# Maofei/loam_velodyne-1

Hardware: AMD Instinct MI355X
Metric: scans/sec (odometry+mapping L-M solve) VLP-16 sweep, 1/2/4/8 MI355X (higher is better)
Workload: dtype fp32 (fp64 JtJ accumulation); 1 GPU; config4: independent VLP-16 problems (SR prev+cur, odometry L-M, mapping L-M); problems_per_gpu=1024, global_batch=1024, split=strong, parallelism=shard1

## Files before the change

### loam_velodyne-1_amd/csrc/dev_common.hpp

```cpp
#ifndef LOAM_DEV_COMMON_HPP
#define LOAM_DEV_COMMON_HPP

#include <hip/hip_runtime.h>
#include <stdint.h>

#define LOAM_HD __host__ __device__ __forceinline__
#define LOAM_D __device__ __forceinline__

#ifdef LOAM_BOUNDS_CHECK
#define LOAM_CHECK(cond, a, b)                                                                      \
  do {                                                                                              \
    if (!(cond)) printf("LOAM_CHECK %s:%d %s (%lld, %lld)\n", __FILE__, __LINE__, #cond, (long long)(a), \
                        (long long)(b));                                                            \
  } while (0)
#else
#define LOAM_CHECK(cond, a, b) ((void)0)
#endif

struct PhaseAcc {
  unsigned long long s0, s1, s2;
  unsigned long long sum[2][12];
};
#ifdef LOAM_PHASES
#define LOAM_PH(...) __VA_ARGS__
// ... 362 lines not shown
    for (int stride = size >> 1; stride > 0; stride >>= 1) {
      for (int t = threadIdx.x; t < (n64 >> 1); t += NT) {
        int lo = 2 * t - (t & (stride - 1));
        int hi = lo + stride;
        bool up = ((lo & size) == 0);
        uint64_t a = k[lo], b = k[hi];
        if ((a > b) == up) { k[lo] = b; k[hi] = a; }
      }
      const int next = stride > 1 ? stride >> 1 : (size << 1 <= n64 ? size : 0);
      if (stride > 64 || next > 64 || next == 0) {
        __syncthreads();
      } else {
        __threadfence_block();
        __builtin_amdgcn_wave_barrier();
      }
    }
  }
}

LOAM_D uint64_t shfl_xor_u64(uint64_t v, int m) {
  const int lo = __shfl_xor((int)(uint32_t)v, m, 64), hi = __shfl_xor((int)(uint32_t)(v >> 32), m, 64);
  return ((uint64_t)(uint32_t)hi << 32) | (uint32_t)lo;
}
template <int E, int S>
LOAM_D void reg_cmpx_intra(uint64_t (&v)[E], int base, int size) {
#pragma unroll
  for (int e = 0; e < E; ++e) {
    if constexpr (S < E) {
      if ((e & S) == 0) {
        const bool up = ((base + e) & size) == 0;
        const uint64_t a = v[e], b = v[e + S];
        const bool sw = (a > b) == up;
        v[e] = sw ? b : a;
        v[e + S] = sw ? a : b;
      }
    }
  }
}
template <int NT, int E, bool WAVE = false>
LOAM_D void reg_bitonic_sort_n(uint64_t* k, int n) {
  static_assert(!WAVE || NT == 64, "a wave sort has 64 lanes");
  const int lane = __lane_id(), tid = WAVE ? lane : (int)threadIdx.x, base = tid * E;
  constexpr int N = NT * E;
  uint64_t v[E];
#pragma unroll
  for (int e = 0; e < E; ++e) {
    const int g = e * NT + tid;
    v[e] = g < n ? k[g] : ~0ull;
  }
  if (!WAVE) __syncthreads();
  for (int size = 2; size <= N; size <<= 1) {
    for (int stride = size >> 1; stride > 0; stride >>= 1) {
      if (stride < E) {
        if (stride == 1) reg_cmpx_intra<E, 1>(v, base, size);
        else if (stride == 2) reg_cmpx_intra<E, 2>(v, base, size);
        else if (stride == 4) reg_cmpx_intra<E, 4>(v, base, size);
        else reg_cmpx_intra<E, 8>(v, base, size);
      } else if (stride < 64 * E) {
        const int m = stride / E;
        const bool lower = (lane & m) == 0;
#pragma unroll
        for (int e = 0; e < E; ++e) {
          const bool up = ((base + e) & size) == 0;
          const uint64_t o = shfl_xor_u64(v[e], m);
          const bool keep_min = lower == up;
          v[e] = keep_min ? (o < v[e] ? o : v[e]) : (o > v[e] ? o : v[e]);
        }
      } else {
        const int m = stride / E;
        const bool lower = (tid & m) == 0;
#pragma unroll
        for (int e = 0; e < E; ++e) k[e * NT + tid] = v[e];
        __syncthreads();
#pragma unroll
        for (int e = 0; e < E; ++e) {
          const bool up = ((base + e) & size) == 0;
          const uint64_t o = k[e * NT + (tid ^ m)];
          const bool keep_min = lower == up;
          v[e] = keep_min ? (o < v[e] ? o : v[e]) : (o > v[e] ? o : v[e]);
        }
        __syncthreads();
      }
    }
  }
  if (WAVE) __builtin_amdgcn_wave_barrier();
#pragma unroll
  for (int e = 0; e < E; ++e)
    if (base + e < n) k[base + e] = v[e];
  if (WAVE) {
    __threadfence_block();
    __builtin_amdgcn_wave_barrier();
  } else {
    __syncthreads();
  }
}
LOAM_D void wave_sort_u64(uint64_t* k, int n) {
  if (n <= 64) reg_bitonic_sort_n<64, 1, true>(k, n);
  else if (n <= 128) reg_bitonic_sort_n<64, 2, true>(k, n);
  else if (n <= 256) reg_bitonic_sort_n<64, 4, true>(k, n);
  else reg_bitonic_sort_n<64, 8, true>(k, n);
}
template <int NT, int EMAX>
LOAM_D void reg_bitonic_sort(uint64_t* k, int n) {
  if (n <= NT || EMAX == 1) reg_bitonic_sort_n<NT, 1>(k, n);
  else if (n <= 2 * NT || EMAX == 2) reg_bitonic_sort_n<NT, (EMAX < 2 ? EMAX : 2)>(k, n);
  else if (n <= 4 * NT || EMAX == 4) reg_bitonic_sort_n<NT, (EMAX < 4 ? EMAX : 4)>(k, n);
  else if (n <= 8 * NT || EMAX == 8) reg_bitonic_sort_n<NT, (EMAX < 8 ? EMAX : 8)>(k, n);
  else reg_bitonic_sort_n<NT, (EMAX < 16 ? EMAX : 16)>(k, n);
}

template <int NT, int E>
LOAM_D int block_radix_sort_kv(uint32_t* ka, uint16_t* va, uint32_t* kb, uint16_t* vb, int n, int nbits,
                               uint32_t* sc) {
  constexpr int NW = NT / 64;
  const int tid = threadIdx.x, lane = __lane_id(), w = tid >> 6;
  int cur = 0;
  for (int shift = 0; shift < nbits; shift += 4) {
    const uint32_t* ks = cur ? kb : ka;
    const uint16_t* vs = cur ? vb : va;
    uint32_t* kd = cur ? ka : kb;
    uint16_t* vd = cur ? va : vb;
    uint32_t k[E];
    uint32_t meta[E];
    uint64_t clo = 0, chi = 0;
#pragma unroll
    for (int e = 0; e < E; ++e) {
      const int g = tid * E + e;
      k[e] = 0;
      meta[e] = 0;
      if (g < n) {
        k[e] = ks[g];
// ... 813 lines not shown
```

### loam_velodyne-1_amd/csrc/engine.hpp

```cpp
#ifndef LOAM_ENGINE_HPP
#define LOAM_ENGINE_HPP

#include <hip/hip_runtime.h>
#include <stdint.h>

#include <cstring>
#include <string>

#include "../../include/loam/loam.h"
#include "imu.hpp"
#include "prof.hpp"

namespace loam {

enum : int {
  ERR_CAP_RING = 1,
  ERR_CAP_ROWS = 2,
  ERR_EMPTY = 4,
  ERR_CAP_MAP = 8,
  ERR_CAP_STACK = 16,
  ERR_VG_BITS = 32,
};

constexpr int kSrThreads = 512;
// ... 50 lines not shown
      if (std::strcmp(key, k.n) == 0) {
        if (read) {
          *read = *k.f;
          return true;
        }
        if (v < k.lo || v > k.hi) return false;
        *k.f = (int)v;
        return true;
      }
    return false;
  }
};

struct SrBuffers {
  int S = 0, cap = 0, R = 0;
  float4* raw = nullptr;
  int* raw_n = nullptr;
  float* tmp_ori = nullptr;
  uint8_t* tmp_sid = nullptr;
  int* tilecnt = nullptr;
  int* tileF = nullptr;
  int* ring_sync = nullptr;
  float* sweep_ori = nullptr;
  float4* full = nullptr;
  int* n_full = nullptr;
  float* curv = nullptr;
  uint8_t* picked = nullptr;
  int* sortind = nullptr;
  int8_t* label = nullptr;
  int* ring_se = nullptr;
  int* st_sharp = nullptr;
  int* st_lsharp = nullptr;
  int* st_flat = nullptr;
  float4* st_lflat = nullptr;
  int* st_cnt = nullptr;
  uint16_t* st_cand = nullptr;
  int* st_ncand = nullptr;
  float4* sharp = nullptr;
  float4* lsharp = nullptr;
  float4* flat = nullptr;
  float4* lflat = nullptr;
  int* cnt = nullptr;
  int* err = nullptr;
  int* sel_big = nullptr;
  int* sel_list = nullptr;
  int* st_loff = nullptr;
// ... 133 lines not shown
```

### loam_velodyne-1_amd/csrc/sr.hip

```cpp
#include <cmath>
#include <type_traits>
#include <vector>

#include "dev_common.hpp"
#include "dev_hooks.h"
#include "engine.hpp"

using namespace loamdev;

namespace loam {

#ifdef LOAM_SR_PHASES
__device__ unsigned long long g_sr_ph[8];
#define SR_PH(k)                                                                  \
  do {                                                                            \
    if (threadIdx.x == 0) {                                                       \
      const unsigned long long now = __builtin_amdgcn_s_memrealtime();            \
      ph_t[k] = now - ph_last;                                                    \
      ph_last = now;                                                              \
    }                                                                             \
  } while (0)
#else
#define SR_PH(k) ((void)0)
#endif

namespace {


LOAM_HD int ring_id(const SrParams& p, float angle) {
  if (p.ring_model == LOAM_RING_LINEAR) {
    const float step = (p.ring_hi - p.ring_lo) / (float)(p.R - 1);
    const float angleID = (angle - p.ring_lo) / step;
    return (int)(angleID + 0.5f);
  }
  int rounded = (int)(D(angle) + (D(angle) < 0.0 ? -0.5 : +0.5));
  return rounded > 0 ? rounded : rounded + (p.R - 1);
}

LOAM_D int ring_of_exact(const SrParams& p, float px, float py, float pz) {
  const float af = atanf(py / sqrtf(px * px + pz * pz)) * 57.2957795f;
  const int lo = ring_id(p, af - 1e-3f), hi = ring_id(p, af + 1e-3f);
  if (lo == hi) return lo;
  return ring_id(p, (float)(atan(D(py) / sqrt(D(px * px + pz * pz))) * 180 / M_PI));
}

#ifndef LOAM_SR_RING_TAB
// ... 510 lines not shown
          T.valid = 1;
        }
      }
    }
    return;
  }
#pragma unroll
  for (int e = 0; e < kRingE; ++e) {
    const int i = t * kRingTile + e * kSrThreads + tid;
    if (sid[e] != 255) {
      const int pos = sh_base[sid[e]] + sh_pre[sid[e]] + sh_wcnt[sid[e]][e * kW + w] + rank[e];
      const float o = (i <= F) ? ori_first(ori[e], startOri) : ori_second(ori[e], endOri);
      const float relTime = (o - startOri) / (endOri - startOri);
      b.full[(size_t)s * b.cap + pos] = make_float4(q[e].y, q[e].z, q[e].x, (float)(sid[e] + 0.1 * D(relTime)));
    }
  }
}

#ifndef LOAM_SR_RING_FUSED
#define LOAM_SR_RING_FUSED 1
#endif
constexpr bool kSrRingFused = LOAM_SR_RING_FUSED;
constexpr int kSrRingFusedMin = 64;
__global__ __launch_bounds__(kSrThreads) void k_sr_ring_fused(SrBuffers b, SrParams p, int rtiles) {
  constexpr int kW = kSrThreads / 64, kSlots = kRingE * kW;
  static_assert(kSlots <= 64 && (kSlots & (kSlots - 1)) == 0, "slot scan width");
  const int tid = threadIdx.x, lane = lane_id(), w = tid >> 6;
  __shared__ int sh_ticket, sh_last, sh_F;
  __shared__ float sh_start, sh_end_raw;
  __shared__ int sh_cnt[64], sh_tot[64], sh_pre[64], sh_base[64];
  __shared__ int sh_wcnt[64][kSlots];
#ifdef LOAM_SR_PHASES
  unsigned long long ph_t[8] = {0}, ph_last = __builtin_amdgcn_s_memrealtime();
#endif
  if (tid == 0) sh_ticket = atomicAdd(&b.ring_sync[0], 1);
  __syncthreads();
  SR_PH(1);
  const int s = sh_ticket / rtiles, t = sh_ticket % rtiles;
  const int n = b.raw_n[s], R = p.R, nt = (n + kRingTile - 1) / kRingTile;
  const int nb = key_bits(R);
  if (t == 0) {
    if (tid < 2 * R) b.ring_se[s * 2 * R + tid] = 0;
    if (tid == 0) b.err[s] = 0;
  }
  if (n <= 0) {
    if (t == 0 && tid == 0) {
      b.n_full[s] = 0;
      b.err[s] |= ERR_EMPTY;
    }
    return;
  }
  if (t >= nt) return;
  const float4* raw = b.raw + (size_t)s * b.cap;
  float4 q[kRingE];
#pragma unroll
  for (int e = 0; e < kRingE; ++e) {
    const int i = t * kRingTile + e * kSrThreads + tid;
    q[e] = i < n ? raw[i] : make_float4(0, 0, 0, 0);
  }
  if (w < 2) {
    int f = -1;
    float4 v = make_float4(0, 0, 0, 0);
    for (int k = 0; k < n; k += 64) {
      const int i = w == 0 ? k + lane : n - 1 - k - lane;
      const bool in = w == 0 ? i < n : i >= 0;
      v = in ? raw[i] : make_float4(0, 0, 0, 0);
      const uint64_t m = __ballot(in && finite3(v));
      if (m) {
        const int src = __ffsll((unsigned long long)m) - 1;
        f = w == 0 ? k + src : n - 1 - k - src;
        v.x = __shfl(v.x, src, 64);
        v.y = __shfl(v.y, src, 64);
        break;
      }
    }
    if (lane == 0) {
      if (w == 0) {
        sh_start = f >= 0 ? -atan2f_fdlibm(v.y, v.x) : 0.0f;
      } else {
        sh_last = f;
        if (f >= 0) sh_end_raw = -atan2f_fdlibm(v.y, v.x);
      }
    }
  }
  __shared__ float4 sh_rtab[kRingTabMax];
  ring_tab_load(p, sh_rtab);
  if (tid < R) sh_cnt[tid] = 0;
  if (tid == 0) sh_F = 0x7fffffff;
  for (int k = tid; k < 64 * kSlots; k += kSrThreads) (&sh_wcnt[0][0])[k] = 0;
  __syncthreads();
  SR_PH(2);
  const float startOri = sh_start;
  float endOri = 0.0f;
  if (sh_last >= 0) {
    endOri = (float)(D(sh_end_raw) + 2 * M_PI);
    if (D(endOri - startOri) > 3 * M_PI) endOri = (float)(D(endOri) - 2 * M_PI);
    else if (D(endOri - startOri) < M_PI) endOri = (float)(D(endOri) + 2 * M_PI);
  }
  if (tid == 0 && t == 0) {
    if (sh_last < 0) b.err[s] |= ERR_EMPTY;
    b.sweep_ori[2 * s] = startOri;
    b.sweep_ori[2 * s + 1] = endOri;
  }
  int sid[kRingE], rank[kRingE];
  float ori[kRingE];
  int Floc = 0x7fffffff;
#pragma unroll
  for (int e = 0; e < kRingE; ++e) {
    const int i = t * kRingTile + e * kSrThreads + tid;
    sid[e] = 255;
    ori[e] = 0.0f;
    if (i < n && finite3(q[e])) {
      const float px = q[e].y, py = q[e].z, pz = q[e].x;
      const int scanID = ring_of(p, sh_rtab, px, py, pz);
      if (scanID >= 0 && scanID <= R - 1) {
        sid[e] = scanID;
        ori[e] = -atan2f_fdlibm(px, pz);
        if (D(ori_first(ori[e], startOri) - startOri) > M_PI) Floc = min(Floc, i);
        atomicAdd(&sh_cnt[scanID], 1);
      }
    }
  }
  Floc = wave_min_i(Floc);
// ... 175 lines not shown
  uint64_t keys[CAP];
  int sidx[SIDX ? CAP : 1];
  uint16_t cand[CAP];
  uint8_t pk[CAP + 16];
  int8_t lab[CAP + 16];
  int se[128];
  int picks[kSharpPerRing + kLessSharpPerRing + kFlatPerRing];
  int scratch[16];
  float red[6][kSelThreads / 64];
  int order[64];
  int nsharp, nlsharp, nflat, ncand, wf, big, loff;
};

#ifndef LOAM_RINGVG_PAD
#define LOAM_RINGVG_PAD 0
#endif
#ifndef LOAM_VG_GATHER
#define LOAM_VG_GATHER 4
#endif
constexpr int kVgGather = LOAM_VG_GATHER;
#ifndef LOAM_RINGVG_HOLD
#define LOAM_RINGVG_HOLD 1
#endif
template <int CAP, bool BIG, typename CandT>
LOAM_D int ring_vg(const float4* pts, int lo, const CandT* cand, int nc, uint64_t* keys, float4* outp, int outcap,
                   float (*red)[kSelThreads / 64], int* scratch, int* err) {
  const int tid = threadIdx.x, lane = lane_id(), w = tid >> 6;
  float mn[3] = {3.4e38f, 3.4e38f, 3.4e38f}, mx[3] = {-3.4e38f, -3.4e38f, -3.4e38f};
  constexpr bool HOLD = !BIG && CAP <= 2048 && LOAM_RINGVG_HOLD;
  constexpr int RH = HOLD ? CAP / kSelThreads : 1;
  float4 held[RH];
  if constexpr (HOLD) {
#pragma unroll
    for (int e = 0; e < RH; ++e) {
      const int t = e * kSelThreads + tid;
      held[e] = t < nc ? pts[lo + cand[t]] : make_float4(0, 0, 0, 0);
    }
#pragma unroll
    for (int e = 0; e < RH; ++e)
      if (e * kSelThreads + tid < nc) {
        const float4 a = held[e];
        mn[0] = fminf(mn[0], a.x); mn[1] = fminf(mn[1], a.y); mn[2] = fminf(mn[2], a.z);
        mx[0] = fmaxf(mx[0], a.x); mx[1] = fmaxf(mx[1], a.y); mx[2] = fmaxf(mx[2], a.z);
      }
  } else {
    for (int t = tid; t < nc; t += kSelThreads) {
      const float4 a = pts[lo + cand[t]];
      mn[0] = fminf(mn[0], a.x); mn[1] = fminf(mn[1], a.y); mn[2] = fminf(mn[2], a.z);
      mx[0] = fmaxf(mx[0], a.x); mx[1] = fmaxf(mx[1], a.y); mx[2] = fmaxf(mx[2], a.z);
    }
  }
  for (int d = 0; d < 3; ++d) {
    mn[d] = wave_min_f_x(mn[d]);
    mx[d] = wave_max_f_x(mx[d]);
    if (lane == 0) { red[d][w] = mn[d]; red[3 + d][w] = mx[d]; }
  }
  __syncthreads();
  for (int d = 0; d < 3; ++d)
    for (int v = 0; v < kSelThreads / 64; ++v) {
      mn[d] = fminf(mn[d], red[d][v]);
      mx[d] = fmaxf(mx[d], red[3 + d][v]);
    }
  __syncthreads();
  int nout = 0;
  if (nc > 0) {
    const float inv = 1.0f / 0.2f;
    if (vg_leaf_too_small(mn, mx, inv)) {
      for (int t = tid; t < nc; t += kSelThreads)
        if (t < outcap) outp[t] = pts[lo + cand[t]];
      nout = nc;
    } else {
      int minb[3], maxb[3];
      for (int d = 0; d < 3; ++d) {
        minb[d] = (int)floorf(mn[d] * inv);
        maxb[d] = (int)floorf(mx[d] * inv);
      }
      const int divx = maxb[0] - minb[0] + 1, divy = maxb[1] - minb[1] + 1;
      const int mul1 = divx, mul2 = divx * divy;
      if constexpr (!BIG) {
        constexpr int NW = kSelThreads / 64;
        int nruns = 0;
        if constexpr (HOLD) {
          static_assert(RH * NW <= 64, "slot prefix over one wave");
          __shared__ uint32_t rs_edge[RH * NW];
          __shared__ int rs_cnt[RH * NW];
          uint32_t idx[RH];
          int ex[RH];
#pragma unroll
          for (int e = 0; e < RH; ++e) {
            const int t = e * kSelThreads + tid;
            idx[e] = 0xffffffffu;
            if (t < nc) {
              const float4 a = held[e];
              const int i0 = (int)(floorf(a.x * inv) - (float)minb[0]);
              const int i1 = (int)(floorf(a.y * inv) - (float)minb[1]);
              const int i2 = (int)(floorf(a.z * inv) - (float)minb[2]);
              idx[e] = (uint32_t)(i0 + i1 * mul1 + i2 * mul2);
            }
            if (lane == 63) rs_edge[e * NW + w] = idx[e];
          }
          __syncthreads();
#pragma unroll
          for (int e = 0; e < RH; ++e) {
            const int t = e * kSelThreads + tid, slot = e * NW + w;
            uint32_t up = (uint32_t)__shfl_up((int)idx[e], 1, 64);
            if (lane == 0 && slot > 0) up = rs_edge[slot - 1];
            const bool head = t < nc && (t == 0 || idx[e] != up);
            const uint64_t m = __ballot(head);
            ex[e] = head ? __popcll(m & lanemask_lt()) : -1;
            if (lane == 0) rs_cnt[slot] = __popcll(m);
          }
          __syncthreads();
          const int c = lane < RH * NW ? rs_cnt[lane] : 0;
          const int incl = wave_incl_scan_x(c);
          nruns = __shfl(incl, RH * NW - 1, 64);
#pragma unroll
          for (int e = 0; e < RH; ++e) {
            const int base = __shfl(incl - c, e * NW + w, 64);
            if (ex[e] >= 0) keys[base + ex[e]] = ((uint64_t)idx[e] << 32) | ((uint32_t)(e * kSelThreads + tid) << 16);
          }
        } else {
        uint32_t* edge = reinterpret_cast<uint32_t*>(&red[0][0]);
        for (int base = 0; base < nc; base += kSelThreads) {
          const int t = base + tid;
          uint32_t idx = 0xffffffffu;
          if (t < nc) {
            float4 a;
            if constexpr (HOLD) {
              a = held[0];
#pragma unroll
              for (int e = 1; e < RH; ++e)
                if (base == e * kSelThreads) a = held[e];
            } else {
              a = pts[lo + cand[t]];
            }
            const int i0 = (int)(floorf(a.x * inv) - (float)minb[0]);
            const int i1 = (int)(floorf(a.y * inv) - (float)minb[1]);
            const int i2 = (int)(floorf(a.z * inv) - (float)minb[2]);
            idx = (uint32_t)(i0 + i1 * mul1 + i2 * mul2);
          }
          uint32_t up = (uint32_t)__shfl_up((int)idx, 1, 64);
          if (lane == 63) edge[w + 1] = idx;
          __syncthreads();
          if (lane == 0) up = edge[w];
          const int head = (t < nc && (t == 0 || idx != up)) ? 1 : 0;
          int tot;
          const int ex = block_excl_scan<kSelThreads>(head, scratch, tot);
          if (head) keys[nruns + ex] = ((uint64_t)idx << 32) | ((uint32_t)t << 16);
          if (tid == kSelThreads - 1) edge[0] = idx;
          nruns += tot;
        }
        }
        __syncthreads();
        constexpr int RE = CAP / kSelThreads;
        uint32_t nxt[RE];
#pragma unroll
        for (int e = 0; e < RE; ++e) {
          const int r = e * kSelThreads + tid;
          nxt[e] = r + 1 < nruns ? (uint32_t)keys[r + 1] >> 16 : (uint32_t)nc;
        }
        __syncthreads();
#pragma unroll
        for (int e = 0; e < RE; ++e) {
          const int r = e * kSelThreads + tid;
          if (r < nruns) keys[r] |= nxt[e] - ((uint32_t)keys[r] >> 16);
        }
        __syncthreads();
        reg_bitonic_sort<kSelThreads, CAP / kSelThreads>(keys, nruns);
        static_assert(RE * NW <= 64, "slot prefix over one wave");
        __shared__ int vs_cnt[RE * NW];
        int vex[RE];
#pragma unroll
        for (int e = 0; e < RE; ++e) {
          const int r = e * kSelThreads + tid;
          const bool head = r < nruns && (r == 0 || (keys[r] >> 32) != (keys[r - 1] >> 32));
          const uint64_t m = __ballot(head);
          vex[e] = head ? __popcll(m & lanemask_lt()) : -1;
          if (lane == 0) vs_cnt[e * NW + w] = __popcll(m);
        }
        __syncthreads();
        const int vc = lane < RE * NW ? vs_cnt[lane] : 0;
        const int vincl = wave_incl_scan_x(vc);
#pragma unroll
        for (int e = 0; e < RE; ++e) {
          const int r = e * kSelThreads + tid;
          const int vbase = __shfl(vincl - vc, e * NW + w, 64);
          if (vex[e] >= 0) {
            const int slot_out = vbase + vex[e];
            const uint32_t vk = (uint32_t)(keys[r] >> 32);
            float sx = 0, sy = 0, sz = 0, si = 0;
            int cnt = 0;
            int rr = r;
            uint32_t kk = (uint32_t)keys[r];
            int m = (int)(kk >> 16), m1 = m + (int)(kk & 0xffffu);
            const int mfirst = m;
            bool more = true;
            while (more) {
              int mi[kVgGather];
#pragma unroll
              for (int u = 0; u < kVgGather; ++u) {
                if (more && m >= m1) {
                  ++rr;
                  if (rr < nruns && (uint32_t)(keys[rr] >> 32) == vk) {
                    kk = (uint32_t)keys[rr];
                    m = (int)(kk >> 16);
                    m1 = m + (int)(kk & 0xffffu);
                  } else {
                    more = false;
                  }
                }
                mi[u] = more ? m++ : -1;
              }
              float4 a[kVgGather];
#pragma unroll
              for (int u = 0; u < kVgGather; ++u) a[u] = pts[lo + cand[mi[u] >= 0 ? mi[u] : mfirst]];
#pragma unroll
              for (int u = 0; u < kVgGather; ++u)
                if (mi[u] >= 0) { sx += a[u].x; sy += a[u].y; sz += a[u].z; si += a[u].w; ++cnt; }
              if (more && m >= m1)
                more = rr + 1 < nruns && (uint32_t)(keys[rr + 1] >> 32) == vk;
            }
            const float fc = (float)cnt;
            if (slot_out < outcap) outp[slot_out] = make_float4(sx / fc, sy / fc, sz / fc, si / fc);
          }
        }
        __syncthreads();
        nout = __shfl(vincl, RE * NW - 1, 64);
      } else
      {
        const int P2c = next_pow2(nc);
        for (int t = tid; t < P2c; t += kSelThreads) {
          uint64_t key = ~0ull;
          if (t < nc) {
            const float4 a = pts[lo + cand[t]];
            int i0 = (int)(floorf(a.x * inv) - (float)minb[0]);
            int i1 = (int)(floorf(a.y * inv) - (float)minb[1]);
            int i2 = (int)(floorf(a.z * inv) - (float)minb[2]);
            uint32_t idx = (uint32_t)(i0 + i1 * mul1 + i2 * mul2);
            key = ((uint64_t)idx << 32) | (uint32_t)t;
          }
          keys[t] = key;
        }
        __syncthreads();
        if constexpr (BIG) block_bitonic_sort<kSelThreads>(keys, P2c);
        else reg_bitonic_sort<kSelThreads, CAP / kSelThreads>(keys, P2c);
        int run = 0;
        for (int base = 0; base < nc; base += kSelThreads) {
          const int t = base + tid;
          const int head = (t < nc && (t == 0 || (keys[t] >> 32) != (keys[t - 1] >> 32))) ? 1 : 0;
          int tot;
// ... 487 lines not shown
    __builtin_amdgcn_wave_barrier();
    for (int base = s0; base < s1; base += 64) {
      const int k = base + lane;
      const bool flag = k < s1 && P.lab[k - wlo] <= 0;
      const uint64_t m = __ballot(flag);
      if (flag) cand[run + __popcll(m & lanemask_lt())] = (uint16_t)(k - lo);
      run += __popcll(m);
    }
    }
#pragma unroll
    for (int k = 0; k < kPickSegRegs; ++k) cra[k] = crb[k];
  }
  __threadfence_block();
  __builtin_amdgcn_wave_barrier();
  const int ns = P.nsharp, nl = P.nlsharp, nf = P.nflat;
  for (int t = lane; t < ns; t += 64) b.st_sharp[(size_t)(s * R + q) * kSharpPerRing + t] = P.picks[t];
  for (int t = lane; t < nl; t += 64) b.st_lsharp[(size_t)(s * R + q) * kLessSharpPerRing + t] = P.picks[kSharpPerRing + t];
  for (int t = lane; t < nf; t += 64)
    b.st_flat[(size_t)(s * R + q) * kFlatPerRing + t] = P.picks[kSharpPerRing + kLessSharpPerRing + t];
  if (lane == 0) { st_cnt[0] = ns; st_cnt[1] = nl; st_cnt[2] = nf; b.st_ncand[s * R + q] = run; }
}

__global__ __launch_bounds__(kSelThreads) void k_sr_ringvg(SrBuffers b, SrParams p) {
  const int q = blockIdx.x, s = blockIdx.y, tid = threadIdx.x, R = p.R;
  const int big = b.sel_big[s], n = b.n_full[s];
  int lo = b.ring_se[s * 2 * R + q], en = b.ring_se[s * 2 * R + R + q];
  const int nc = min(b.st_ncand[s * R + q], kPickCap);
  if (big != 0 || n <= 0) return;
  if (q == 0) lo = 5;
  if (q == R - 1) en = n - 5;
  if (lo > en - 1) return;
  __shared__ uint64_t keys[kPickCap];
  __shared__ uint16_t cand[kPickCap];
  __shared__ float red[6][kSelThreads / 64];
  __shared__ int scratch[16];
  const uint16_t* cg = b.st_cand + (size_t)(s * R + q) * kRingCap;
  for (int t = tid; t < nc; t += kSelThreads) cand[t] = cg[t];
  __syncthreads();
  const int nout = ring_vg<kPickCap, false>(b.full + (size_t)s * b.cap, lo, cand, nc, keys,
                                            b.st_lflat + (size_t)s * R * kRingCap + q * kRingCap, kRingCap, red,
                                            scratch, b.err + s);
  if (tid == 0) b.st_cnt[(size_t)(s * R + q) * 4 + 3] = nout;
}

LOAM_D void sel_init(const SrBuffers& b, int s, int n) {
  for (int k = threadIdx.x; k < n; k += blockDim.x) {
    b.sortind[(size_t)s * b.cap + k] = k;
    b.label[(size_t)s * b.cap + k] = 0;
  }
  __threadfence_block();
  __syncthreads();
}

template <int CAP, int MODE>
__global__ __launch_bounds__(kSelThreads) __attribute__((amdgpu_waves_per_eu(MODE == 0 ? 6 : 1))) void k_sr_select(SrBuffers b, SrParams p) {
  constexpr bool BIG = MODE == 2;
  const int tid = threadIdx.x, R = p.R;
  constexpr bool SIDX = MODE != 0;
  __shared__ SelShared<CAP, SIDX> sh;
  const int nlist = MODE == 0 ? b.S : b.sel_list[MODE - 1];
  const int* list = b.sel_list + 2 + (MODE == 2 ? b.S : 0);
  for (int i = BIG ? blockIdx.x : blockIdx.y; i < nlist; i += BIG ? gridDim.x : gridDim.y) {
    const int s = MODE == 0 ? i : list[i];
    const int q = BIG ? 0 : blockIdx.x;
// ... 187 lines not shown
    job.dbase[c] = dbase[c];
  }
  job.tile0[kPackClouds] = tiles;
  if (tiles == 0) return hipSuccess;
  const long long items = (long long)tiles * nj;
  if (items > 0x7fffffffLL) return hipErrorInvalidValue;
  hipLaunchKernelGGL(k_sr_pack, dim3((unsigned)std::min<long long>(items, kPackGridMax)), dim3(kPackThreads), 0, st, b,
                     job, table, dst);
  return hipGetLastError();
}

hipError_t sr_alloc(SrBuffers& b, int S, int cap, int R) {
  DevAlloc A;
  b.S = S; b.cap = cap; b.R = R;
  const size_t n = (size_t)S * cap;
  A(&b.raw, n * sizeof(float4));
  A(&b.raw_n, S * sizeof(int));
  A(&b.tmp_ori, n * sizeof(float));
  A(&b.tmp_sid, n);
  A(&b.tilecnt, (size_t)S * b.ntiles() * R * sizeof(int));
  A(&b.tileF, (size_t)S * b.ntiles() * sizeof(int));
  A(&b.ring_sync, sizeof(int));
  A(&b.sweep_ori, (size_t)S * 2 * sizeof(float));
  A(&b.full, n * sizeof(float4));
  A(&b.n_full, S * sizeof(int));
  A(&b.curv, n * sizeof(float));
  A(&b.picked, n);
  A(&b.sortind, n * sizeof(int));
  A(&b.label, n);
  A(&b.ring_se, (size_t)S * 2 * R * sizeof(int));
  A(&b.st_sharp, (size_t)S * R * kSharpPerRing * sizeof(int));
  A(&b.st_lsharp, (size_t)S * R * kLessSharpPerRing * sizeof(int));
  A(&b.st_flat, (size_t)S * R * kFlatPerRing * sizeof(int));
  A(&b.st_lflat, (size_t)S * R * kRingCap * sizeof(float4));
  A(&b.st_cnt, (size_t)S * R * 4 * sizeof(int));
  A(&b.st_cand, (size_t)S * R * kRingCap * sizeof(uint16_t));
  A(&b.st_ncand, (size_t)S * R * sizeof(int));
  A(&b.sharp, (size_t)S * R * kSharpPerRing * sizeof(float4));
  A(&b.lsharp, (size_t)S * R * kLessSharpPerRing * sizeof(float4));
  A(&b.flat, (size_t)S * R * kFlatPerRing * sizeof(float4));
  A(&b.lflat, n * sizeof(float4));
  A(&b.cnt, (size_t)S * 4 * sizeof(int));
  A(&b.err, S * sizeof(int));
  A(&b.sel_big, S * sizeof(int));
  A(&b.sel_list, (2 + 2 * (size_t)S) * sizeof(int));
  A(&b.st_loff, (size_t)S * R * sizeof(int));
// ... 75 lines not shown
  t = SrRingTab();
  const std::vector<float4> tab = sr_ring_tab_build(p, t.a0, t.ainv);
  if (tab.empty()) return hipSuccess;
  hipError_t e = hipMalloc((void**)&t.dev, tab.size() * sizeof(float4));
  if (e != hipSuccess) {
    t.dev = nullptr;
    return e;
  }
  e = hipMemcpy(t.dev, tab.data(), tab.size() * sizeof(float4), hipMemcpyHostToDevice);
  if (e != hipSuccess) {
    sr_ring_tab_free(t);
    return e;
  }
  t.n = (int)tab.size();
  return hipSuccess;
}

void sr_ring_tab_free(SrRingTab& t) {
  if (t.dev) HIPCHK(hipFree(t.dev));
  t = SrRingTab();
}

void sr_free(SrBuffers& b) {
  void* ptrs[] = {b.raw, b.raw_n, b.tmp_ori, b.tmp_sid, b.tilecnt, b.tileF, b.ring_sync, b.sweep_ori, b.full, b.n_full, b.curv,
                  b.picked, b.sortind, b.label, b.ring_se, b.st_sharp, b.st_lsharp, b.st_flat,
                  b.st_lflat, b.st_cnt, b.st_cand, b.st_ncand, b.sharp, b.lsharp, b.flat, b.lflat, b.cnt, b.err, b.sel_big, b.sel_list, b.st_loff, b.big_keys, b.big_sidx, b.big_cand};
  for (void* q : ptrs)
    if (q) HIPCHK(hipFree(q));
  b = SrBuffers();
}

int sr_ring_fused_capacity() {
  static int cap[64];
  int dev = 0;
  if (hipGetDevice(&dev) != hipSuccess || dev < 0 || dev >= 64) return 0;
  if (cap[dev] == 0) {
    int per_cu = 0, cus = 0;
    if (hipOccupancyMaxActiveBlocksPerMultiprocessor(&per_cu, k_sr_ring_fused, kSrThreads, 0) != hipSuccess ||
        hipDeviceGetAttribute(&cus, hipDeviceAttributeMultiprocessorCount, dev) != hipSuccess)
      per_cu = cus = 0;
    cap[dev] = std::max(1, per_cu * cus);
  }
  return cap[dev];
}

void sr_launch(const SrBuffers& b, const SrParams& p, hipStream_t st, Prof* prof, hipEvent_t sorted) {
  auto mark = [&](const char* n) { if (prof) prof->mark(n); };
  const bool lanes_imu = p.imu && p.imu_lane;
  if (p.imu && !lanes_imu) {
    HIPCHK(hipMemsetAsync(b.ring_se, 0, (size_t)b.S * 2 * b.R * sizeof(int), st));
    HIPCHK(hipMemsetAsync(b.err, 0, (size_t)b.S * sizeof(int), st));
  }
  mark("sr_memset");
  if (lanes_imu) {
    const int rtiles = (b.cap + kRingTile - 1) / kRingTile;
    hipLaunchKernelGGL(k_sr_ring_count<true>, dim3(rtiles, b.S), dim3(kSrThreads), 0, st, b, p);
    hipLaunchKernelGGL(k_sr_ring_scatter<true>, dim3(rtiles, b.S), dim3(kSrThreads), 0, st, b, p);
  } else if (p.imu) {
    hipLaunchKernelGGL(k_sr_ring_sort<true>, dim3(b.S), dim3(kSrThreads), 0, st, b, p);
  } else {
    const int rtiles = (b.cap + kRingTile - 1) / kRingTile;
    if (kSrRingFused && b.S >= kSrRingFusedMin && 2 * rtiles <= sr_ring_fused_capacity()) {
      HIPCHK(hipMemsetAsync(b.ring_sync, 0, sizeof(int), st));
      HIPCHK(hipMemsetAsync(b.tilecnt, 0xff, (size_t)b.S * rtiles * b.R * sizeof(int), st));
      HIPCHK(hipMemsetAsync(b.tileF, 0xff, (size_t)b.S * rtiles * sizeof(int), st));
      hipLaunchKernelGGL(k_sr_ring_fused, dim3(rtiles * b.S), dim3(kSrThreads), 0, st, b, p, rtiles);
    } else {
      hipLaunchKernelGGL(k_sr_ring_count<false>, dim3(rtiles, b.S), dim3(kSrThreads), 0, st, b, p);
      hipLaunchKernelGGL(k_sr_ring_scatter<false>, dim3(rtiles, b.S), dim3(kSrThreads), 0, st, b, p);
    }
  }
  mark("k_sr_ring_sort");
  if (sorted) HIPCHK(hipEventRecord(sorted, st));
  hipLaunchKernelGGL(k_sr_features, dim3((b.cap + kFeatSpan - 1) / kFeatSpan, b.S), dim3(kFeatTile), 0,
                     st, b, p);
  mark("k_sr_features");
  hipLaunchKernelGGL(k_sr_pick, dim3((b.R + kPickWaves - 1) / kPickWaves, b.S), dim3(64 * kPickWaves), 0, st, b, p);
  hipLaunchKernelGGL(k_sr_ringvg, dim3(b.R, b.S), dim3(kSelThreads), LOAM_RINGVG_PAD, st, b, p);
  hipLaunchKernelGGL((k_sr_select<kRingCap, 1>), dim3(b.R, std::min(b.S, kSelListGrid)), dim3(kSelThreads), 0, st, b, p);
  hipLaunchKernelGGL((k_sr_select<16, 2>), dim3(kBigSlots), dim3(kSelThreads), 0, st, b, p);
  mark("k_sr_select");
  hipLaunchKernelGGL(k_sr_compact, dim3(b.R, b.S), dim3(256), 0, st, b, p);
  mark("k_sr_compact");
}

namespace {
__global__ __launch_bounds__(256) void k_dev_sr_ring_of(SrParams p, const float4* pts, int n, int* ring, int* exact,
                                                         int* fast) {
// ... 38 lines not shown
  if (e == hipSuccess) e = hipMemcpy(dpts, pts, (size_t)n * sizeof(float4), hipMemcpyHostToDevice);
  if (e == hipSuccess) {
    tab.fill(p);
    hipLaunchKernelGGL(k_dev_sr_ring_of, dim3((n + 255) / 256), dim3(256), 0, nullptr, p, dpts, n, dout, dout + n,
                       dout + 2 * (size_t)n);
    e = hipGetLastError();
  }
  if (e == hipSuccess) e = hipMemcpy(ring, dout, (size_t)n * sizeof(int), hipMemcpyDeviceToHost);
  if (e == hipSuccess) e = hipMemcpy(exact, dout + n, (size_t)n * sizeof(int), hipMemcpyDeviceToHost);
  if (e == hipSuccess) e = hipMemcpy(fast, dout + 2 * (size_t)n, (size_t)n * sizeof(int), hipMemcpyDeviceToHost);
  if (dpts) (void)hipFree(dpts);
  if (dout) (void)hipFree(dout);
  sr_ring_tab_free(tab);
  return e == hipSuccess ? LOAM_OK : (nomem ? LOAM_E_NOMEM : LOAM_E_HIP);
}

#ifdef LOAM_SR_PHASES
extern "C" int loam_debug_phases_sr(unsigned long long* out) {
  if (hipDeviceSynchronize() != hipSuccess) return -1;
  if (hipMemcpyFromSymbol(out, HIP_SYMBOL(loam::g_sr_ph), sizeof(loam::g_sr_ph)) != hipSuccess) return -1;
  const unsigned long long zero[8] = {0};
  return hipMemcpyToSymbol(HIP_SYMBOL(loam::g_sr_ph), zero, sizeof(zero)) == hipSuccess ? 0 : -1;
}
#endif
```

Before: 97260 scans/s.

## Add ring prep kernel, sweep-ends precompute, 32-bit voxel sort keys, register candidates

A new per-scan prep kernel replaces three memsets and computes each sweep's first and last finite point orientation once. The fused ring kernel then reads these ends instead of every tile searching for them, and issues its raw loads earlier. Ring voxel-grid downsampling now uses packed 32-bit sort keys with a run-start table when the voxel count fits, which halves the bitonic sort width. Candidate indices are also preloaded into registers before the early return. Together these add a launch and some code complexity in exchange for fewer memsets, less redundant scanning and a cheaper shared-memory sort.

```diff
diff --git a/loam_velodyne-1_amd/csrc/dev_common.hpp b/loam_velodyne-1_amd/csrc/dev_common.hpp
--- a/loam_velodyne-1_amd/csrc/dev_common.hpp
+++ b/loam_velodyne-1_amd/csrc/dev_common.hpp
@@ -408,14 +408,16 @@
   const int lo = __shfl_xor((int)(uint32_t)v, m, 64), hi = __shfl_xor((int)(uint32_t)(v >> 32), m, 64);
   return ((uint64_t)(uint32_t)hi << 32) | (uint32_t)lo;
 }
-template <int E, int S>
-LOAM_D void reg_cmpx_intra(uint64_t (&v)[E], int base, int size) {
+LOAM_D uint64_t shfl_xor_key(uint64_t v, int m) { return shfl_xor_u64(v, m); }
+LOAM_D uint32_t shfl_xor_key(uint32_t v, int m) { return (uint32_t)__shfl_xor((int)v, m, 64); }
+template <int E, int S, typename K>
+LOAM_D void reg_cmpx_intra(K (&v)[E], int base, int size) {
 #pragma unroll
   for (int e = 0; e < E; ++e) {
     if constexpr (S < E) {
       if ((e & S) == 0) {
         const bool up = ((base + e) & size) == 0;
-        const uint64_t a = v[e], b = v[e + S];
+        const K a = v[e], b = v[e + S];
         const bool sw = (a > b) == up;
         v[e] = sw ? b : a;
         v[e + S] = sw ? a : b;
@@ -423,32 +425,32 @@
     }
   }
 }
-template <int NT, int E, bool WAVE = false>
-LOAM_D void reg_bitonic_sort_n(uint64_t* k, int n) {
+template <int NT, int E, bool WAVE = false, typename K = uint64_t>
+LOAM_D void reg_bitonic_sort_n(K* k, int n) {
   static_assert(!WAVE || NT == 64, "a wave sort has 64 lanes");
   const int lane = __lane_id(), tid = WAVE ? lane : (int)threadIdx.x, base = tid * E;
   constexpr int N = NT * E;
-  uint64_t v[E];
+  K v[E];
 #pragma unroll
   for (int e = 0; e < E; ++e) {
     const int g = e * NT + tid;
-    v[e] = g < n ? k[g] : ~0ull;
+    v[e] = g < n ? k[g] : (K)~(K)0;
   }
   if (!WAVE) __syncthreads();
   for (int size = 2; size <= N; size <<= 1) {
     for (int stride = size >> 1; stride > 0; stride >>= 1) {
       if (stride < E) {
-        if (stride == 1) reg_cmpx_intra<E, 1>(v, base, size);
-        else if (stride == 2) reg_cmpx_intra<E, 2>(v, base, size);
-        else if (stride == 4) reg_cmpx_intra<E, 4>(v, base, size);
-        else reg_cmpx_intra<E, 8>(v, base, size);
+        if (stride == 1) reg_cmpx_intra<E, 1, K>(v, base, size);
+        else if (stride == 2) reg_cmpx_intra<E, 2, K>(v, base, size);
+        else if (stride == 4) reg_cmpx_intra<E, 4, K>(v, base, size);
+        else reg_cmpx_intra<E, 8, K>(v, base, size);
       } else if (stride < 64 * E) {
         const int m = stride / E;
         const bool lower = (lane & m) == 0;
 #pragma unroll
         for (int e = 0; e < E; ++e) {
           const bool up = ((base + e) & size) == 0;
-          const uint64_t o = shfl_xor_u64(v[e], m);
+          const K o = shfl_xor_key(v[e], m);
           const bool keep_min = lower == up;
           v[e] = keep_min ? (o < v[e] ? o : v[e]) : (o > v[e] ? o : v[e]);
         }
@@ -461,7 +463,7 @@
 #pragma unroll
         for (int e = 0; e < E; ++e) {
           const bool up = ((base + e) & size) == 0;
-          const uint64_t o = k[e * NT + (tid ^ m)];
+          const K o = k[e * NT + (tid ^ m)];
           const bool keep_min = lower == up;
           v[e] = keep_min ? (o < v[e] ? o : v[e]) : (o > v[e] ? o : v[e]);
         }
@@ -486,13 +488,13 @@
   else if (n <= 256) reg_bitonic_sort_n<64, 4, true>(k, n);
   else reg_bitonic_sort_n<64, 8, true>(k, n);
 }
-template <int NT, int EMAX>
-LOAM_D void reg_bitonic_sort(uint64_t* k, int n) {
-  if (n <= NT || EMAX == 1) reg_bitonic_sort_n<NT, 1>(k, n);
-  else if (n <= 2 * NT || EMAX == 2) reg_bitonic_sort_n<NT, (EMAX < 2 ? EMAX : 2)>(k, n);
-  else if (n <= 4 * NT || EMAX == 4) reg_bitonic_sort_n<NT, (EMAX < 4 ? EMAX : 4)>(k, n);
-  else if (n <= 8 * NT || EMAX == 8) reg_bitonic_sort_n<NT, (EMAX < 8 ? EMAX : 8)>(k, n);
-  else reg_bitonic_sort_n<NT, (EMAX < 16 ? EMAX : 16)>(k, n);
+template <int NT, int EMAX, typename K>
+LOAM_D void reg_bitonic_sort(K* k, int n) {
+  if (n <= NT || EMAX == 1) reg_bitonic_sort_n<NT, 1, false, K>(k, n);
+  else if (n <= 2 * NT || EMAX == 2) reg_bitonic_sort_n<NT, (EMAX < 2 ? EMAX : 2), false, K>(k, n);
+  else if (n <= 4 * NT || EMAX == 4) reg_bitonic_sort_n<NT, (EMAX < 4 ? EMAX : 4), false, K>(k, n);
+  else if (n <= 8 * NT || EMAX == 8) reg_bitonic_sort_n<NT, (EMAX < 8 ? EMAX : 8), false, K>(k, n);
+  else reg_bitonic_sort_n<NT, (EMAX < 16 ? EMAX : 16), false, K>(k, n);
 }
 
 template <int NT, int E>
diff --git a/loam_velodyne-1_amd/csrc/engine.hpp b/loam_velodyne-1_amd/csrc/engine.hpp
--- a/loam_velodyne-1_amd/csrc/engine.hpp
+++ b/loam_velodyne-1_amd/csrc/engine.hpp
@@ -96,6 +96,7 @@
   int* tileF = nullptr;
   int* ring_sync = nullptr;
   float* sweep_ori = nullptr;
+  int4* sweep_ends = nullptr;
   float4* full = nullptr;
   int* n_full = nullptr;
   float* curv = nullptr;
diff --git a/loam_velodyne-1_amd/csrc/sr.hip b/loam_velodyne-1_amd/csrc/sr.hip
--- a/loam_velodyne-1_amd/csrc/sr.hip
+++ b/loam_velodyne-1_amd/csrc/sr.hip
@@ -12,6 +12,7 @@
 
 #ifdef LOAM_SR_PHASES
 __device__ unsigned long long g_sr_ph[8];
+__device__ unsigned long long g_vg_ph[8];
 #define SR_PH(k)                                                                  \
   do {                                                                            \
     if (threadIdx.x == 0) {                                                       \
@@ -20,8 +21,12 @@
       ph_last = now;                                                              \
     }                                                                             \
   } while (0)
+#define SR_PH_PARAM , unsigned long long ph0 = 0
+#define SR_PH_ARG(x) , x
 #else
 #define SR_PH(k) ((void)0)
+#define SR_PH_PARAM
+#define SR_PH_ARG(x)
 #endif
 
 namespace {
@@ -578,12 +583,59 @@
 #endif
 constexpr bool kSrRingFused = LOAM_SR_RING_FUSED;
 constexpr int kSrRingFusedMin = 64;
+#ifndef LOAM_SR_ENDS_ONCE
+#define LOAM_SR_ENDS_ONCE 1
+#endif
+constexpr int kPrepThreads = 128;
+__global__ __launch_bounds__(kPrepThreads) void k_sr_ring_prep(SrBuffers b, int R, int rtiles) {
+  const int s = blockIdx.x, tid = threadIdx.x, lane = lane_id(), w = tid >> 6;
+  const int n = b.raw_n[s];
+  const float4* raw = b.raw + (size_t)s * b.cap;
+  __shared__ int sh_last;
+  __shared__ float sh_start, sh_end_raw;
+  if (tid == 0) { sh_last = -1; sh_start = 0.0f; sh_end_raw = 0.0f; }
+  int* tc = b.tilecnt + (size_t)s * rtiles * R;
+  for (int k = tid; k < rtiles * R; k += kPrepThreads) tc[k] = -1;
+  for (int k = tid; k < rtiles; k += kPrepThreads) b.tileF[(size_t)s * rtiles + k] = -1;
+  if (s == 0 && tid == 0) b.ring_sync[0] = 0;
+  __syncthreads();
+  if (LOAM_SR_ENDS_ONCE) {
+    int f = -1;
+    float4 v = make_float4(0, 0, 0, 0);
+    for (int k = 0; k < n; k += 64) {
+      const int i = w == 0 ? k + lane : n - 1 - k - lane;
+      const bool in = w == 0 ? i < n : i >= 0;
+      v = in ? raw[i] : make_float4(0, 0, 0, 0);
+      const uint64_t m = __ballot(in && finite3(v));
+      if (m) {
+        const int src = __ffsll((unsigned long long)m) - 1;
+        f = w == 0 ? k + src : n - 1 - k - src;
+        v.x = __shfl(v.x, src, 64);
+        v.y = __shfl(v.y, src, 64);
+        break;
+      }
+    }
+    if (lane == 0) {
+      if (w == 0) {
+        sh_start = f >= 0 ? -atan2f_fdlibm(v.y, v.x) : 0.0f;
+      } else {
+        sh_last = f;
+        if (f >= 0) sh_end_raw = -atan2f_fdlibm(v.y, v.x);
+      }
+    }
+    __syncthreads();
+    if (tid == 0) b.sweep_ends[s] = make_int4(sh_last, __float_as_int(sh_start), __float_as_int(sh_end_raw), 0);
+  }
+}
 __global__ __launch_bounds__(kSrThreads) void k_sr_ring_fused(SrBuffers b, SrParams p, int rtiles) {
   constexpr int kW = kSrThreads / 64, kSlots = kRingE * kW;
   static_assert(kSlots <= 64 && (kSlots & (kSlots - 1)) == 0, "slot scan width");
   const int tid = threadIdx.x, lane = lane_id(), w = tid >> 6;
-  __shared__ int sh_ticket, sh_last, sh_F;
+  __shared__ int sh_ticket, sh_F;
+#if !LOAM_SR_ENDS_ONCE
+  __shared__ int sh_last;
   __shared__ float sh_start, sh_end_raw;
+#endif
   __shared__ int sh_cnt[64], sh_tot[64], sh_pre[64], sh_base[64];
   __shared__ int sh_wcnt[64][kSlots];
 #ifdef LOAM_SR_PHASES
@@ -592,8 +644,26 @@
   if (tid == 0) sh_ticket = atomicAdd(&b.ring_sync[0], 1);
   __syncthreads();
   SR_PH(1);
-  const int s = sh_ticket / rtiles, t = sh_ticket % rtiles;
+#if LOAM_SR_ENDS_ONCE
+  const int ticket = __builtin_amdgcn_readfirstlane(sh_ticket);
+#else
+  const int ticket = sh_ticket;
+#endif
+  const int s = ticket / rtiles, t = ticket % rtiles;
+  const float4* raw = b.raw + (size_t)s * b.cap;
+#if LOAM_SR_ENDS_ONCE
+  const int n = b.raw_n[s];
+  const int4 ends = b.sweep_ends[s];
+  float4 q[kRingE];
+#pragma unroll
+  for (int e = 0; e < kRingE; ++e) {
+    const int i = t * kRingTile + e * kSrThreads + tid;
+    q[e] = i < b.cap ? raw[i] : make_float4(0, 0, 0, 0);
+  }
+  const int R = p.R, nt = (n + kRingTile - 1) / kRingTile;
+#else
   const int n = b.raw_n[s], R = p.R, nt = (n + kRingTile - 1) / kRingTile;
+#endif
   const int nb = key_bits(R);
   if (t == 0) {
     if (tid < 2 * R) b.ring_se[s * 2 * R + tid] = 0;
@@ -607,7 +677,10 @@
     return;
   }
   if (t >= nt) return;
-  const float4* raw = b.raw + (size_t)s * b.cap;
+#if LOAM_SR_ENDS_ONCE
+  const int last = ends.x;
+  const float startOri = __int_as_float(ends.y), end_raw = __int_as_float(ends.z);
+#else
   float4 q[kRingE];
 #pragma unroll
   for (int e = 0; e < kRingE; ++e) {
@@ -639,6 +712,7 @@
       }
     }
   }
+#endif
   __shared__ float4 sh_rtab[kRingTabMax];
   ring_tab_load(p, sh_rtab);
   if (tid < R) sh_cnt[tid] = 0;
@@ -646,15 +720,18 @@
   for (int k = tid; k < 64 * kSlots; k += kSrThreads) (&sh_wcnt[0][0])[k] = 0;
   __syncthreads();
   SR_PH(2);
-  const float startOri = sh_start;
+#if !LOAM_SR_ENDS_ONCE
+  const float startOri = sh_start, end_raw = sh_end_raw;
+  const int last = sh_last;
+#endif
   float endOri = 0.0f;
-  if (sh_last >= 0) {
-    endOri = (float)(D(sh_end_raw) + 2 * M_PI);
+  if (last >= 0) {
+    endOri = (float)(D(end_raw) + 2 * M_PI);
     if (D(endOri - startOri) > 3 * M_PI) endOri = (float)(D(endOri) - 2 * M_PI);
     else if (D(endOri - startOri) < M_PI) endOri = (float)(D(endOri) + 2 * M_PI);
   }
   if (tid == 0 && t == 0) {
-    if (sh_last < 0) b.err[s] |= ERR_EMPTY;
+    if (last < 0) b.err[s] |= ERR_EMPTY;
     b.sweep_ori[2 * s] = startOri;
     b.sweep_ori[2 * s + 1] = endOri;
   }
@@ -876,10 +953,19 @@
 #ifndef LOAM_RINGVG_HOLD
 #define LOAM_RINGVG_HOLD 1
 #endif
+#ifndef LOAM_RINGVG_K32
+#define LOAM_RINGVG_K32 1
+#endif
+#ifndef LOAM_RINGVG_CREG
+#define LOAM_RINGVG_CREG 1
+#endif
 template <int CAP, bool BIG, typename CandT>
-LOAM_D int ring_vg(const float4* pts, int lo, const CandT* cand, int nc, uint64_t* keys, float4* outp, int outcap,
-                   float (*red)[kSelThreads / 64], int* scratch, int* err) {
+LOAM_D int ring_vg(const float4* pts, int lo, CandT* cand, int nc, uint64_t* keys, float4* outp, int outcap,
+                   float (*red)[kSelThreads / 64], int* scratch, int* err, const CandT* creg = nullptr SR_PH_PARAM) {
   const int tid = threadIdx.x, lane = lane_id(), w = tid >> 6;
+#ifdef LOAM_SR_PHASES
+  unsigned long long ph_t[8] = {0}, ph_last = ph0 ? ph0 : __builtin_amdgcn_s_memrealtime();
+#endif
   float mn[3] = {3.4e38f, 3.4e38f, 3.4e38f}, mx[3] = {-3.4e38f, -3.4e38f, -3.4e38f};
   constexpr bool HOLD = !BIG && CAP <= 2048 && LOAM_RINGVG_HOLD;
   constexpr int RH = HOLD ? CAP / kSelThreads : 1;
@@ -888,7 +974,12 @@
 #pragma unroll
     for (int e = 0; e < RH; ++e) {
       const int t = e * kSelThreads + tid;
-      held[e] = t < nc ? pts[lo + cand[t]] : make_float4(0, 0, 0, 0);
+      if (creg) {
+        held[e] = t < nc ? pts[lo + creg[e]] : make_float4(0, 0, 0, 0);
+        if (t < nc) cand[t] = creg[e];
+      } else {
+        held[e] = t < nc ? pts[lo + cand[t]] : make_float4(0, 0, 0, 0);
+      }
     }
 #pragma unroll
     for (int e = 0; e < RH; ++e)
@@ -919,6 +1010,7 @@
   int nout = 0;
   if (nc > 0) {
     const float inv = 1.0f / 0.2f;
+    SR_PH(1);
     if (vg_leaf_too_small(mn, mx, inv)) {
       for (int t = tid; t < nc; t += kSelThreads)
         if (t < outcap) outp[t] = pts[lo + cand[t]];
@@ -934,6 +1026,11 @@
       if constexpr (!BIG) {
         constexpr int NW = kSelThreads / 64;
         int nruns = 0;
+        constexpr bool K32 = HOLD && LOAM_RINGVG_K32;
+        [[maybe_unused]] int rb = 0;
+        [[maybe_unused]] bool k32 = false;
+        uint32_t* const key32 = reinterpret_cast<uint32_t*>(keys);
+        uint16_t* const first = reinterpret_cast<uint16_t*>(key32 + CAP);
         if constexpr (HOLD) {
           static_assert(RH * NW <= 64, "slot prefix over one wave");
           __shared__ uint32_t rs_edge[RH * NW];
@@ -968,10 +1065,27 @@
           const int c = lane < RH * NW ? rs_cnt[lane] : 0;
           const int incl = wave_incl_scan_x(c);
           nruns = __shfl(incl, RH * NW - 1, 64);
+          if constexpr (K32) {
+            rb = nruns > 1 ? 32 - __clz(nruns - 1) : 0;
+            const uint64_t nvox = (uint64_t)divx * (uint64_t)divy * (uint64_t)(maxb[2] - minb[2] + 1);
+            k32 = nvox <= (1ull << (32 - rb));
+          }
+          if (k32) {
+#pragma unroll
+            for (int e = 0; e < RH; ++e) {
+              const int j = __shfl(incl - c, e * NW + w, 64) + ex[e];
+              if (ex[e] >= 0) {
+                key32[j] = (idx[e] << rb) | (uint32_t)j;
+                first[j] = (uint16_t)(e * kSelThreads + tid);
+              }
+            }
+            if (tid == 0) first[nruns] = (uint16_t)nc;
+          } else {
 #pragma unroll
           for (int e = 0; e < RH; ++e) {
             const int base = __shfl(incl - c, e * NW + w, 64);
             if (ex[e] >= 0) keys[base + ex[e]] = ((uint64_t)idx[e] << 32) | ((uint32_t)(e * kSelThreads + tid) << 16);
+          }
           }
         } else {
         uint32_t* edge = reinterpret_cast<uint32_t*>(&red[0][0]);
@@ -1007,6 +1121,7 @@
         }
         __syncthreads();
         constexpr int RE = CAP / kSelThreads;
+        if (!k32) {
         uint32_t nxt[RE];
 #pragma unroll
         for (int e = 0; e < RE; ++e) {
@@ -1020,66 +1135,99 @@
           if (r < nruns) keys[r] |= nxt[e] - ((uint32_t)keys[r] >> 16);
         }
         __syncthreads();
-        reg_bitonic_sort<kSelThreads, CAP / kSelThreads>(keys, nruns);
+        }
+        SR_PH(2);
+        if (k32) reg_bitonic_sort<kSelThreads, CAP / kSelThreads>(key32, nruns);
+        else reg_bitonic_sort<kSelThreads, CAP / kSelThreads>(keys, nruns);
+        SR_PH(3);
         static_assert(RE * NW <= 64, "slot prefix over one wave");
         __shared__ int vs_cnt[RE * NW];
-        int vex[RE];
-#pragma unroll
-        for (int e = 0; e < RE; ++e) {
-          const int r = e * kSelThreads + tid;
-          const bool head = r < nruns && (r == 0 || (keys[r] >> 32) != (keys[r - 1] >> 32));
-          const uint64_t m = __ballot(head);
-          vex[e] = head ? __popcll(m & lanemask_lt()) : -1;
-          if (lane == 0) vs_cnt[e * NW + w] = __popcll(m);
+        auto means = [&](auto wide) {
+          constexpr bool K = !decltype(wide)::value;
+          auto vox = [&](int r) -> uint32_t {
+            if constexpr (K) return key32[r] >> rb;
+            else return (uint32_t)(keys[r] >> 32);
+          };
+          auto span = [&](int r, int& m, int& m1) {
+            if constexpr (K) {
+              const int j = (int)(key32[r] & ((1u << rb) - 1u));
+              m = first[j];
+              m1 = first[j + 1];
+            } else {
+              const uint32_t kk = (uint32_t)keys[r];
+              m = (int)(kk >> 16);
+              m1 = m + (int)(kk & 0xffffu);
+            }
+          };
+          int vex[RE];
+#pragma unroll
+          for (int e = 0; e < RE; ++e) {
+            const int r = e * kSelThreads + tid;
+            const bool head = r < nruns && (r == 0 || vox(r) != vox(r - 1));
+            const uint64_t m = __ballot(head);
+            vex[e] = head ? __popcll(m & lanemask_lt()) : -1;
+            if (lane == 0) vs_cnt[e * NW + w] = __popcll(m);
+          }
+          __syncthreads();
+          SR_PH(4);
+          const int vc = lane < RE * NW ? vs_cnt[lane] : 0;
+          const int vincl = wave_incl_scan_x(vc);
+#pragma unroll
+          for (int e = 0; e < RE; ++e) {
+            const int r = e * kSelThreads + tid;
+            const int vbase = __shfl(vincl - vc, e * NW + w, 64);
+            if (vex[e] >= 0) {
+              const int slot_out = vbase + vex[e];
+              const uint32_t vk = vox(r);
+              float sx = 0, sy = 0, sz = 0, si = 0;
+              int cnt = 0;
+              int rr = r, m, m1;
+              span(r, m, m1);
+              const int mfirst = m;
+              bool more = true;
+              while (more) {
+                int mi[kVgGather];
+#pragma unroll
+                for (int u = 0; u < kVgGather; ++u) {
+                  if (more && m >= m1) {
+                    ++rr;
+                    if (rr < nruns && vox(rr) == vk) span(rr, m, m1);
+                    else more = false;
+                  }
+                  mi[u] = more ? m++ : -1;
+                }
+                float4 a[kVgGather];
+#pragma unroll
+                for (int u = 0; u < kVgGather; ++u) a[u] = pts[lo + cand[mi[u] >= 0 ? mi[u] : mfirst]];
+#pragma unroll
+                for (int u = 0; u < kVgGather; ++u)
+                  if (mi[u] >= 0) { sx += a[u].x; sy += a[u].y; sz += a[u].z; si += a[u].w; ++cnt; }
+                if (more && m >= m1)
+                  more = rr + 1 < nruns && vox(rr + 1) == vk;
+              }
+              const float fc = (float)cnt;
+              if (slot_out < outcap) outp[slot_out] = make_float4(sx / fc, sy / fc, sz / fc, si / fc);
+            }
+          }
+          __syncthreads();
+          SR_PH(5);
+          nout = __shfl(vincl, RE * NW - 1, 64);
+        };
+        if constexpr (K32) {
+          if (k32) means(std::false_type{});
+          else means(std::true_type{});
+        } else {
+          means(std::true_type{});
         }
-        __syncthreads();
-        const int vc = lane < RE * NW ? vs_cnt[lane] : 0;
-        const int vincl = wave_incl_scan_x(vc);
-#pragma unroll
-        for (int e = 0; e < RE; ++e) {
-          const int r = e * kSelThreads + tid;
-          const int vbase = __shfl(vincl - vc, e * NW + w, 64);
-          if (vex[e] >= 0) {
-            const int slot_out = vbase + vex[e];
-            const uint32_t vk = (uint32_t)(keys[r] >> 32);
-            float sx = 0, sy = 0, sz = 0, si = 0;
-            int cnt = 0;
-            int rr = r;
-            uint32_t kk = (uint32_t)keys[r];
-            int m = (int)(kk >> 16), m1 = m + (int)(kk & 0xffffu);
-            const int mfirst = m;
-            bool more = true;
-            while (more) {
-              int mi[kVgGather];
-#pragma unroll
-              for (int u = 0; u < kVgGather; ++u) {
-                if (more && m >= m1) {
-                  ++rr;
-                  if (rr < nruns && (uint32_t)(keys[rr] >> 32) == vk) {
-                    kk = (uint32_t)keys[rr];
-                    m = (int)(kk >> 16);
-                    m1 = m + (int)(kk & 0xffffu);
-                  } else {
-                    more = false;
-                  }
-                }
-                mi[u] = more ? m++ : -1;
-              }
-              float4 a[kVgGather];
-#pragma unroll
-              for (int u = 0; u < kVgGather; ++u) a[u] = pts[lo + cand[mi[u] >= 0 ? mi[u] : mfirst]];
-#pragma unroll
-              for (int u = 0; u < kVgGather; ++u)
-                if (mi[u] >= 0) { sx += a[u].x; sy += a[u].y; sz += a[u].z; si += a[u].w; ++cnt; }
-              if (more && m >= m1)
-                more = rr + 1 < nruns && (uint32_t)(keys[rr + 1] >> 32) == vk;
-            }
-            const float fc = (float)cnt;
-            if (slot_out < outcap) outp[slot_out] = make_float4(sx / fc, sy / fc, sz / fc, si / fc);
+#ifdef LOAM_SR_PHASES
+        if constexpr (HOLD)
+          if (tid == 0) {
+            atomicAdd(&g_vg_ph[0], 1ull);
+            for (int k = 1; k < 6; ++k) atomicAdd(&g_vg_ph[k], ph_t[k]);
+            atomicAdd(&g_vg_ph[6], k32 ? 1ull : 0ull);
+            atomicAdd(&g_vg_ph[7], (unsigned long long)nruns);
           }
-        }
-        __syncthreads();
-        nout = __shfl(vincl, RE * NW - 1, 64);
+#endif
       } else
       {
         const int P2c = next_pow2(nc);
@@ -1613,10 +1761,20 @@
 }
 
 __global__ __launch_bounds__(kSelThreads) void k_sr_ringvg(SrBuffers b, SrParams p) {
+#ifdef LOAM_SR_PHASES
+  const unsigned long long ph0 = __builtin_amdgcn_s_memrealtime();
+#endif
   const int q = blockIdx.x, s = blockIdx.y, tid = threadIdx.x, R = p.R;
   const int big = b.sel_big[s], n = b.n_full[s];
   int lo = b.ring_se[s * 2 * R + q], en = b.ring_se[s * 2 * R + R + q];
   const int nc = min(b.st_ncand[s * R + q], kPickCap);
+  const uint16_t* cg = b.st_cand + (size_t)(s * R + q) * kRingCap;
+#if LOAM_RINGVG_CREG
+  static_assert(kPickCap <= kRingCap, "candidate row");
+  uint16_t creg[kPickCap / kSelThreads];
+#pragma unroll
+  for (int e = 0; e < kPickCap / kSelThreads; ++e) creg[e] = cg[e * kSelThreads + tid];
+#endif
   if (big != 0 || n <= 0) return;
   if (q == 0) lo = 5;
   if (q == R - 1) en = n - 5;
@@ -1625,12 +1783,16 @@
   __shared__ uint16_t cand[kPickCap];
   __shared__ float red[6][kSelThreads / 64];
   __shared__ int scratch[16];
-  const uint16_t* cg = b.st_cand + (size_t)(s * R + q) * kRingCap;
+#if LOAM_RINGVG_CREG
+  const uint16_t* cr = creg;
+#else
+  const uint16_t* cr = nullptr;
   for (int t = tid; t < nc; t += kSelThreads) cand[t] = cg[t];
   __syncthreads();
+#endif
   const int nout = ring_vg<kPickCap, false>(b.full + (size_t)s * b.cap, lo, cand, nc, keys,
                                             b.st_lflat + (size_t)s * R * kRingCap + q * kRingCap, kRingCap, red,
-                                            scratch, b.err + s);
+                                            scratch, b.err + s, cr SR_PH_ARG(ph0));
   if (tid == 0) b.st_cnt[(size_t)(s * R + q) * 4 + 3] = nout;
 }
 
@@ -1864,6 +2026,7 @@
   A(&b.tileF, (size_t)S * b.ntiles() * sizeof(int));
   A(&b.ring_sync, sizeof(int));
   A(&b.sweep_ori, (size_t)S * 2 * sizeof(float));
+  A(&b.sweep_ends, (size_t)S * sizeof(int4));
   A(&b.full, n * sizeof(float4));
   A(&b.n_full, S * sizeof(int));
   A(&b.curv, n * sizeof(float));
@@ -1985,7 +2148,7 @@
 }
 
 void sr_free(SrBuffers& b) {
-  void* ptrs[] = {b.raw, b.raw_n, b.tmp_ori, b.tmp_sid, b.tilecnt, b.tileF, b.ring_sync, b.sweep_ori, b.full, b.n_full, b.curv,
+  void* ptrs[] = {b.raw, b.raw_n, b.tmp_ori, b.tmp_sid, b.tilecnt, b.tileF, b.ring_sync, b.sweep_ori, b.sweep_ends, b.full, b.n_full, b.curv,
                   b.picked, b.sortind, b.label, b.ring_se, b.st_sharp, b.st_lsharp, b.st_flat,
                   b.st_lflat, b.st_cnt, b.st_cand, b.st_ncand, b.sharp, b.lsharp, b.flat, b.lflat, b.cnt, b.err, b.sel_big, b.sel_list, b.st_loff, b.big_keys, b.big_sidx, b.big_cand};
   for (void* q : ptrs)
@@ -2024,9 +2187,7 @@
   } else {
     const int rtiles = (b.cap + kRingTile - 1) / kRingTile;
     if (kSrRingFused && b.S >= kSrRingFusedMin && 2 * rtiles <= sr_ring_fused_capacity()) {
-      HIPCHK(hipMemsetAsync(b.ring_sync, 0, sizeof(int), st));
-      HIPCHK(hipMemsetAsync(b.tilecnt, 0xff, (size_t)b.S * rtiles * b.R * sizeof(int), st));
-      HIPCHK(hipMemsetAsync(b.tileF, 0xff, (size_t)b.S * rtiles * sizeof(int), st));
+      hipLaunchKernelGGL(k_sr_ring_prep, dim3(b.S), dim3(kPrepThreads), 0, st, b, b.R, rtiles);
       hipLaunchKernelGGL(k_sr_ring_fused, dim3(rtiles * b.S), dim3(kSrThreads), 0, st, b, p, rtiles);
     } else {
       hipLaunchKernelGGL(k_sr_ring_count<false>, dim3(rtiles, b.S), dim3(kSrThreads), 0, st, b, p);
@@ -2111,4 +2272,10 @@
   const unsigned long long zero[8] = {0};
   return hipMemcpyToSymbol(HIP_SYMBOL(loam::g_sr_ph), zero, sizeof(zero)) == hipSuccess ? 0 : -1;
 }
+extern "C" int loam_debug_phases_ringvg(unsigned long long* out) {
+  if (hipDeviceSynchronize() != hipSuccess) return -1;
+  if (hipMemcpyFromSymbol(out, HIP_SYMBOL(loam::g_vg_ph), sizeof(loam::g_vg_ph)) != hipSuccess) return -1;
+  const unsigned long long zero[8] = {0};
+  return hipMemcpyToSymbol(HIP_SYMBOL(loam::g_vg_ph), zero, sizeof(zero)) == hipSuccess ? 0 : -1;
+}
 #endif
```

Result: faster. 99190 scans/s, median of 6 (+2.0%).
